# rjagerman/glint

Measured on AMD Instinct MI355X. Metric: device-resident push scatter-add GB/s (and % HBM peak) at 1/2/4/8 GPUs, higher is better.
Workload: dtype f64; 1 GPU; north star: dense contiguous-range push scatter-add, 2^30-key Double vector per GPU (BASELINE.json north_star's 1-GPU target configuration); keys_per_gpu=1073741824, key_dtype=i64, parallelism=range-sharded x1, no exchange

## Files before the change

### glint_amd/csrc/glint_bin.hip

```cpp
#include "glint_device.h"
#include "glint_host.h"

#include <atomic>
#include <cstring>
#include <type_traits>

namespace glint {

#ifndef GLINT_SLAB_BITS
#define GLINT_SLAB_BITS 12
#endif
constexpr int kSlabBits = GLINT_SLAB_BITS;
constexpr int kSlab = 1 << kSlabBits;
constexpr int kMaxDigit = 1024;
#ifndef GLINT_PART_TPB
#define GLINT_PART_TPB 1024
#endif
constexpr int kATPB = GLINT_PART_TPB;
#ifndef GLINT_PART_PER
#define GLINT_PART_PER 4
#endif
constexpr int kAPer = GLINT_PART_PER;
#ifndef GLINT_PART_PER_PLAIN
#define GLINT_PART_PER_PLAIN 8
// ... 264 lines not shown
  const u64 b = ctl->bad;
  if (b == 0ull) {
    if (threadIdx.x == 0) *gate = 0ull;
    return;
  }
  for (u32 x = threadIdx.x; x < nb; x += 256) T[x] = 0;
  if (threadIdx.x == 0) {
    *gate = b;
    ctl->cancel = 1u;
    ctl->brk_enc = 0u;
    bc->tail = 0u;
  }
}

constexpr int kHotSlots = 2048;
constexpr int kHotSample = 16384;
constexpr int kHotRun = 128;
constexpr int kHotRuns = kHotSample / kHotRun;
constexpr int kHotCount = 16384;
constexpr int kHotTPB = 1024;

__device__ __forceinline__ u32 hot_slot(u32 a) { return hot_mix(a) & (kHotSlots - 1); }



template <bool MAT>
__global__ __launch_bounds__(kHotTPB) void bin_hot_pick_kernel(const i64* __restrict__ keys,
                                                               const int32_t* __restrict__ cols, i64 n,
                                                               PartDesc part, const LaunchCtl* lctl, u32 ntiles,
                                                               int from_break, u32 min_count,
                                                               u32* __restrict__ hot_tags) {
  __shared__ u32 ck[kHotCount];
  __shared__ u32 cc[kHotCount];
  __shared__ unsigned long long best[kHotSlots];
  const int tid = threadIdx.x;
  for (int i = tid; i < kHotCount; i += kHotTPB) {
    ck[i] = kEmptySlot;
    cc[i] = 0;
  }
  for (int i = tid; i < kHotSlots; i += kHotTPB) best[i] = 0ull;
  __syncthreads();
  const i64 r0 = tail_start(lctl, ntiles, from_break, n);
  const i64 m = n - r0;
  if (m > 0) {
    const i64 ns = min((i64)kHotSample, m);
    const i64 run_stride = m >= (i64)kHotSample ? m / kHotRuns : kHotRun;
    auto rec_of = [&](i64 sidx) { return r0 + (sidx / kHotRun) * run_stride + (sidx % kHotRun); };
    constexpr int kBatch = 16;
    for (i64 s0 = 0; s0 < ns; s0 += (i64)kBatch * kHotTPB) {
      i64 k[kBatch];
      int32_t c[kBatch];
#pragma unroll
      for (int j = 0; j < kBatch; ++j) {
        const i64 i = rec_of(min(s0 + (i64)j * kHotTPB + tid, ns - 1));
        k[j] = keys[i];
        c[j] = MAT ? cols[i] : 0;
      }
#pragma unroll
      for (int j = 0; j < kBatch; ++j) {
        i64 a64;
        if (s0 + (i64)j * kHotTPB + tid >= ns || !rec_addr<MAT>(part, k[j], c[j], a64)) continue;
        const u32 a = (u32)a64;
        u32 h = hot_mix(a * 0x9E3779B1u) & (kHotCount - 1);
        for (int probe = 0; probe < 64; ++probe) {
          const u32 prev = atomicCAS(&ck[h], kEmptySlot, a);
          if (prev == kEmptySlot || prev == a) {
            atomicAdd(&cc[h], 1u);
            break;
          }
          h = (h + 1) & (kHotCount - 1);
        }
      }
    }
  }
  __syncthreads();
  for (int h = tid; h < kHotCount; h += kHotTPB)
    if (cc[h] >= min_count) atomicMax(&best[hot_slot(ck[h])], ((unsigned long long)cc[h] << 32) | ck[h]);
  __syncthreads();
  for (int i = tid; i < kHotSlots; i += kHotTPB) hot_tags[i] = best[i] ? (u32)best[i] : kEmptySlot;
}

template <typename A> __device__ __forceinline__ A hot_zero() { return A(0); }
template <> __device__ __forceinline__ double hot_zero<double>() { return -0.0; }
template <typename A> __device__ __forceinline__ bool hot_untouched(A x) { return x == A(0); }
template <> __device__ __forceinline__ bool hot_untouched<double>(double x) {
  return __double_as_longlong(x) == (long long)0x8000000000000000ull;
}
__device__ __forceinline__ void hot_flush(double* p, double x) { gadd(p, x); }
__device__ __forceinline__ void hot_flush(float* p, double x) { gadd(p, (float)x); }
__device__ __forceinline__ void hot_flush(long long* p, long long x) { gadd(p, x); }
__device__ __forceinline__ void hot_flush(int* p, int x) { gadd(p, x); }

template <typename A, int P>
__device__ __forceinline__ u32 part_emit(const u32 (&ad)[P], const A (&va)[P], u32 valid, const BinGeom& g,
                                         u32* dcnt, u32* gcnt, u32* st_a, A* st_v, const BufOut& ctb, u32 ctcol,
                                         u32 ctstride, u32* __restrict__ out_a, A* __restrict__ out_v, PhaseClock& ph,
                                         int pb) {
  const int tid = threadIdx.x;
  u32 rank[P];
#pragma unroll
  for (int j = 0; j < P; ++j)
    if (valid & (1u << j)) rank[j] = atomicAdd(&dcnt[bucket_of(ad[j], g)], 1u);
  __syncthreads();
  ph.mark(pb);
  const u32 total = block_scan<kATPB, 1>(
      g.nb, [&](u32 d) { return dcnt[d]; },
      [&](u32 d, u32 excl) {
        gcnt[d] = dcnt[d];
        dcnt[d] = excl;
      });
  ph.mark(pb + 1);
  static_assert(kATPB <= kMaxDigit, "one chunk-table entry per thread");
  bput(ctb, ((u32)tid * ctstride + ctcol) * 4u, (u32)tid < g.nb, dcnt[tid] | (gcnt[tid] << 16));
#pragma unroll
  for (int j = 0; j < P; ++j) {
    if (valid & (1u << j)) {
      const u32 p = dcnt[bucket_of(ad[j], g)] + rank[j];
      st_a[p] = ad[j];
      st_v[p] = va[j];
    }
  }
  __syncthreads();
  ph.mark(pb + 2);
  const RecOut<u32> oa{buf_out(out_a, total * 4u)};
  const RecOut<A> ov{buf_out(out_v, total * (u32)sizeof(A))};
#pragma unroll
  for (int j = 0; j < P; ++j) {
    if ((u32)(j * kATPB) >= total) break;
    const u32 p = tid + j * kATPB;
    const bool on = p < total;
    oa.put(p, on, st_a[p]);
    ov.put(p, on, st_v[p]);
  }
  __syncthreads();
  ph.mark(pb + 3);
  for (u32 d = tid; d < g.nb; d += kATPB) dcnt[d] = 0;
  __syncthreads();
  ph.mark(pb + 4);
  return total;
}

__device__ __forceinline__ void part_next_header(const BinGeom& g, BinCtl* next_bc, u32* __restrict__ next_T,
                                                 LaunchCtl* next_ctl) {
  const int tid = threadIdx.x;
  for (u32 b = tid; b < kMaxDigit; b += kATPB) {
    next_T[b] = 0;
    next_T[kMaxDigit + b] = 0;
  }
  if (tid < (int)(sizeof(BinCtl) / 4)) reinterpret_cast<u32*>(next_bc)[tid] = 0;
  if (next_ctl && tid == 0) {
    next_ctl->brk_enc = 0u;
    next_ctl->nonaffine = 0u;
    next_ctl->cancel = 0u;
    next_ctl->bad = 0ull;
  }
}

__device__ __forceinline__ u32 bucket_items(u32 t, u32 item) { return max(1u, (t + item - 1) / item); }

constexpr int kWideHashBits = 20;
constexpr int kWideRunsPerWg = 8;
constexpr int kWideSampleWgs = 256;

template <bool MAT>
__global__ __launch_bounds__(256) void bin_hot_sample_kernel(const i64* __restrict__ keys, const int32_t* __restrict__ cols,
                                                             i64 n, PartDesc part, const LaunchCtl* lctl, u32 ntiles,
                                                             int from_break, u32* __restrict__ gkey,
                                                             u32* __restrict__ gcnt) {
  constexpr int kLocal = 2048;
  __shared__ u32 lk[kLocal], lc[kLocal];
  const int tid = threadIdx.x;
  for (int i = tid; i < kLocal; i += 256) {
    lk[i] = kEmptySlot;
    lc[i] = 0;
  }
  __syncthreads();
  const i64 r0 = tail_start(lctl, ntiles, from_break, n);
  const i64 m = n - r0;
  const i64 runs = (i64)kWideSampleWgs * kWideRunsPerWg;
  if (m > 0) {
    const i64 stride = m >= runs * kHotRun ? m / runs : kHotRun;
    constexpr int kPer = kWideRunsPerWg * kHotRun / 256;
#pragma unroll
    for (int j = 0; j < kPer; ++j) {
      const int s = j * 256 + tid;
      const i64 run = (i64)blockIdx.x * kWideRunsPerWg + s / kHotRun;
      const i64 i = r0 + run * stride + s % kHotRun;
      if (i >= n) continue;
      i64 a64;
      if (!rec_addr<MAT>(part, keys[i], MAT ? cols[i] : 0, a64)) continue;
      const u32 a = (u32)a64;
      u32 h = hot_mix(a * 0x9E3779B1u) & (kLocal - 1);
      for (int probe = 0; probe < 64; ++probe) {
        const u32 prev = atomicCAS(&lk[h], kEmptySlot, a);
        if (prev == kEmptySlot || prev == a) {
          atomicAdd(&lc[h], 1u);
          break;
        }
        h = (h + 1) & (kLocal - 1);
      }
    }
  }
  __syncthreads();
  constexpr u32 kMask = (1u << kWideHashBits) - 1u;
  for (int i = tid; i < kLocal; i += 256) {
    const u32 a = lk[i];
    if (a == kEmptySlot) continue;
    u32 h = hot_mix(a) & kMask;
    for (int probe = 0; probe < 64; ++probe) {
      const u32 prev = atomicCAS(&gkey[h], kEmptySlot, a);
      if (prev == kEmptySlot || prev == a) {
        atomicAdd(&gcnt[h], lc[i]);
        break;
      }
      h = (h + 1) & kMask;
    }
  }
}

__global__ __launch_bounds__(256) void bin_hot_select_kernel(u32* __restrict__ gkey, u32* __restrict__ gcnt,
                                                             u32 min_count, unsigned long long* __restrict__ best) {
  const u32 i = blockIdx.x * 256u + threadIdx.x;
  const u32 a = gkey[i], c = gcnt[i];
  gkey[i] = kEmptySlot;
  gcnt[i] = 0;
  if (a != kEmptySlot && c >= min_count) atomicMax(&best[wide_slot(a)], ((unsigned long long)c << 32) | a);
}

constexpr int kRedSlots = 64, kRedTPB = 1024, kRedGroups = kRedTPB / kRedSlots;
template <typename V>
__device__ __forceinline__ void hot_reduce_block(u32 blk, const unsigned long long* __restrict__ best, u32 G,
                                                 const typename LdsAcc<V>::T* __restrict__ partial,
                                                 V* __restrict__ data, const LaunchCtl* gated) {
  typedef typename LdsAcc<V>::T A;
  if (gated && gated->cancel) return;
  __shared__ A gs[kRedGroups][kRedSlots];
  __shared__ u32 gany[kRedGroups][kRedSlots];
  const int tid = threadIdx.x, ls = tid % kRedSlots, grp = tid / kRedSlots;
  const u32 sl = blk * (u32)kRedSlots + (u32)ls;
  const u32 per = (G + kRedGroups - 1) / kRedGroups;
  const u32 w0 = grp * per, w1 = min(G, w0 + per);
  A sum = hot_zero<A>();
  u32 any = 0;
  constexpr int kUnroll = 8;
  for (u32 w = w0; w < w1; w += kUnroll) {
    A x[kUnroll];
#pragma unroll
    for (int j = 0; j < kUnroll; ++j) x[j] = partial[(size_t)min(w + (u32)j, w1 - 1u) * kWideSlots + sl];
#pragma unroll
    for (int j = 0; j < kUnroll; ++j) {
      if (w + (u32)j < w1 && !hot_untouched<A>(x[j])) {
        sum = any ? vadd(sum, x[j]) : x[j];
        any = 1;
      }
    }
  }
  gs[grp][ls] = sum;
  gany[grp][ls] = any;
  __syncthreads();
  if (grp != 0) return;
  const unsigned long long b = best[sl];
  if (!b) return;
  A tot = hot_zero<A>();
  bool seen = false;
  for (int q = 0; q < kRedGroups; ++q) {
    if (!gany[q][ls]) continue;
    tot = seen ? vadd(tot, gs[q][ls]) : gs[q][ls];
    seen = true;
  }
  const u32 a = (u32)b;
  if (seen) data[a] = acc_add(data[a], tot);
}

#ifndef GLINT_PART_WAVES
#define GLINT_PART_WAVES 4
#endif
template <typename V, bool MAT, bool HOT, int KIND, bool VALIDATE, int PER = kAPer>
__global__ __launch_bounds__(kATPB) __attribute__((amdgpu_waves_per_eu(HOT ? 4 : GLINT_PART_WAVES))) void bin_part_kernel(
    const i64* __restrict__ keys, const int32_t* __restrict__ cols, const V* __restrict__ vals, i64 n, PartDesc part,
    const LaunchCtl* lctl, u32 ntiles, int from_break, BinGeom g, u32* __restrict__ addr_out,
    typename LdsAcc<V>::T* __restrict__ val_out, ErrState* err, BinCtl* bc, u32* __restrict__ ct, u32 ctstride,
    const unsigned long long* __restrict__ hot_best, typename LdsAcc<V>::T* __restrict__ hot_partial,
    BinCtl* next_bc, u32* __restrict__ next_T, LaunchCtl* vctl, LaunchCtl* next_ctl) {
  typedef typename LdsAcc<V>::T A;
  constexpr int kChunk = kATPB * PER;
  __shared__ u32 dcnt[kMaxDigit], gcnt[kMaxDigit];
  __shared__ u32 st_a[kChunk];
  __shared__ A st_v[kChunk];
  constexpr int kHS = HOT ? kWideSlots : 1;
  __shared__ u32 htag[kHS];
  __shared__ A hacc[kHS];
  const int tid = threadIdx.x;
  const u32 w = blockIdx.x;
  const i64 r0 = tail_start(lctl, ntiles, from_break, n);
  const i64 nchunks = (n - r0 + kChunk - 1) / kChunk;
  constexpr int kAhead = HOT ? 2 : kPartAhead;
  if constexpr (HOT) {
    for (int sl = tid; sl < kWideSlots; sl += kATPB) {
      const unsigned long long b = hot_best[sl];
      htag[sl] = b ? (u32)b : kEmptySlot;
      hacc[sl] = hot_zero<A>();
    }
  }
  for (u32 d = tid; d < g.nb; d += kATPB) dcnt[d] = 0;
  if (w == 0) part_next_header(g, next_bc, next_T, next_ctl);
  __syncthreads();
// ... 1351 lines not shown
```

### glint_amd/csrc/glint_gpu.hip

```cpp
#include "glint_kernels.h"
#include "../../include/glint_gpu.h"
#include "glint_device.h"

#include <mutex>
#include <vector>
#include <utility>
#include <new>
#include <chrono>
#include <cstring>
#include <sched.h>
#include <time.h>
#include <cstdio>
#include <algorithm>
#include <cstdlib>

namespace glint {

template <bool MAT> struct AddrT { typedef int32_t T; };
template <> struct AddrT<true> { typedef i64 T; };

template <bool MAT, int KIND = -1>
__device__ __forceinline__ bool rec_addr_t(const PartDesc& p, i64 key, int32_t col, typename AddrT<MAT>::T& addr) {
  i64 ad;
  const bool ok = rec_addr<MAT, KIND>(p, key, col, ad);
  addr = (typename AddrT<MAT>::T)ad;
  return ok;
}

template <bool MAT, bool FULL, int KIND>
__device__ __forceinline__ bool check_tile(const i64* __restrict__ keys, const int32_t* __restrict__ cols, i64 n,
                                           const PartDesc& part, LaunchCtl* ctl, i64* __restrict__ desc,
                                           u32 ntiles, u32 t, int lane, bool validate, bool read_all) {
  typedef typename AddrT<MAT>::T A;
  const i64 pbase = (i64)t * (kTile / 2);
  K2 k[kPPT];
  C2 c[kPPT];
#pragma unroll
  for (int j = 0; j < kPPT; ++j) {
    const i64 p = pbase + lane + (i64)j * 64;
    const i64 r = 2 * p;
    if (FULL || r + 1 < n) {
      k[j] = __builtin_nontemporal_load(reinterpret_cast<const K2*>(keys) + p);
      if (MAT) c[j] = __builtin_nontemporal_load(reinterpret_cast<const C2*>(cols) + p);
    } else {
      k[j] = K2{r < n ? keys[r] : 0, 0};
      if (MAT) c[j] = C2{r < n ? cols[r] : 0, 0};
    }
  }
  const i64 r_first = 2 * pbase;
  const i64 kb = r_first > 0 ? keys[r_first - 1] : 0;
  const int32_t cb = (MAT && r_first > 0) ? cols[r_first - 1] : 0;
  const u32 brk = __builtin_amdgcn_readfirstlane(ld_relaxed(&ctl->brk_enc));
  const bool after = brk != 0u && ntiles - brk < t;
  if (!read_all && after) return false;
  A before = 0;
  if (r_first > 0) rec_addr_t<MAT, KIND>(part, kb, cb, before);
  bool mono = true, affine = true;
  A a_first = 0;
  A last = before;
#pragma unroll
  for (int j = 0; j < kPPT; ++j) {
    const i64 r = 2 * (pbase + lane + (i64)j * 64);
    const bool h0 = FULL || r < n, h1 = FULL || r + 1 < n;
    A a0, a1;
    const bool o0 = rec_addr_t<MAT, KIND>(part, k[j].x, MAT ? c[j].x : 0, a0);
    const bool o1 = rec_addr_t<MAT, KIND>(part, k[j].y, MAT ? c[j].y : 0, a1);
    if (j == 0) a_first = __shfl(a0, 0);
    if (h1) mono = mono && (a1 > a0);
    A prev = __shfl_up(a1, 1);
    if (lane == 0) prev = last;
    if (h0 && r > 0) mono = mono && (a0 > prev);
    last = __shfl(a1, 63);
    const A off = (A)(r - r_first);
    affine = affine && (!h0 || (o0 && a0 == a_first + off)) && (!h1 || (o1 && a1 == a_first + off + 1));
    if (validate) {
      const bool b0 = h0 && (!o0 || !key_in_part<KIND>(part, k[j].x));
      const bool b1 = h1 && (!o1 || !key_in_part<KIND>(part, k[j].y));
      if (b0 || b1) atomicMax(&ctl->bad, ~(u64)(b0 ? r : r + 1));
    }
  }
  const bool any_bad = __any(!mono);
  const bool all_affine = __all(affine);
  if (lane == 0 && !after) {
    if (any_bad) {
      if (ld_relaxed(&ctl->brk_enc) < ntiles - t) atomicMax(&ctl->brk_enc, ntiles - t);
    } else {
      desc[t] = all_affine ? (i64)a_first : kNotAffine;
      const bool linked = all_affine && (r_first == 0 || (i64)a_first == (i64)before + 1);
      if (!linked && ld_relaxed(&ctl->nonaffine) == 0u) atomicOr(&ctl->nonaffine, 1u);
    }
  }
  return true;
}

template <bool MAT, int KIND>
__global__ __launch_bounds__(kTPB) void push_check_kernel(const i64* __restrict__ keys,
                                                          const int32_t* __restrict__ cols, i64 n,
                                                          PartDesc part, LaunchCtl* ctl, LaunchCtl* next,
                                                          i64* __restrict__ desc, u32 ntiles, u32 t_begin,
                                                          u32 t_end, int validate) {
  const int lane = threadIdx.x & 63;
  if (t_begin == 0 && blockIdx.x == 0 && threadIdx.x == 0) {
    next->brk_enc = 0u;
    next->nonaffine = 0u;
    next->cancel = 0u;
    next->bad = 0ull;
  }
  if (ctl->cancel) return;
  const u32 w0 = blockIdx.x * (kTPB / 64) + (threadIdx.x >> 6);
  const u32 nw = gridDim.x * (kTPB / 64);
  for (u32 t = t_begin + w0; t < t_end; t += nw) {
    const bool full = 2 * ((i64)t * (kTile / 2)) + kTile <= n;
    const bool go = full ? check_tile<MAT, true, KIND>(keys, cols, n, part, ctl, desc, ntiles, t, lane, validate != 0,
                                                       validate == 1)
                         : check_tile<MAT, false, KIND>(keys, cols, n, part, ctl, desc, ntiles, t, lane, validate != 0,
                                                        validate == 1);
    if (!go) return;
  }
}

template <typename V, bool MAT, bool FULL>
__device__ __forceinline__ void apply_affine(const PushArgs<V>& a, i64 pbase, i64 base, int lane) {
  typedef typename Vec2<V>::T V2;
  const i64 n = a.n;
  const i64 r_first = 2 * pbase;
  V2 v[kPPT], d[kPPT];
  if ((base & 1) == 0) {
    V2* dp = reinterpret_cast<V2*>(a.data + base);
#pragma unroll
    for (int j = 0; j < kPPT; ++j) {
      const i64 q = lane + (i64)j * 64;
      if (FULL || 2 * (pbase + q) + 1 < n) {
        v[j] = __builtin_nontemporal_load(reinterpret_cast<const V2*>(a.vals) + pbase + q);
        d[j] = dp[q];
      }
    }
#pragma unroll
    for (int j = 0; j < kPPT; ++j) {
      const i64 q = lane + (i64)j * 64;
      const i64 r = 2 * (pbase + q);
      if (FULL || r + 1 < n) dp[q] = as2<V>(vadd((V)d[j].x, (V)v[j].x), vadd((V)d[j].y, (V)v[j].y));
      else if (r < n) a.data[base + (r - r_first)] = vadd(a.data[base + (r - r_first)], a.vals[r]);
    }
  } else {
#pragma unroll
    for (int j = 0; j < kPPT; ++j) {
      const i64 p = pbase + lane + (i64)j * 64;
      const i64 r = 2 * p;
      const i64 e = base + (r - r_first);
      if (FULL || r + 1 < n) {
        v[j] = __builtin_nontemporal_load(reinterpret_cast<const V2*>(a.vals) + p);
        d[j] = as2<V>(a.data[e], a.data[e + 1]);
      } else {
        v[j] = as2<V>(r < n ? a.vals[r] : V(0), V(0));
        d[j] = as2<V>(r < n ? a.data[e] : V(0), V(0));
      }
    }
#pragma unroll
    for (int j = 0; j < kPPT; ++j) {
      const i64 r = 2 * (pbase + lane + (i64)j * 64);
      const i64 e = base + (r - r_first);
      if (FULL || r < n) a.data[e] = vadd((V)d[j].x, (V)v[j].x);
      if (FULL || r + 1 < n) a.data[e + 1] = vadd((V)d[j].y, (V)v[j].y);
    }
  }
}

template <typename V, bool MAT, bool FULL>
__device__ __forceinline__ void apply_general(const PushArgs<V>& a, i64 pbase, int lane) {
  typedef typename Vec2<V>::T V2;
  typedef typename AddrT<MAT>::T A;
  const i64 n = a.n;
  K2 k[kPPT];
  C2 c[kPPT];
  V2 v[kPPT];
#pragma unroll
  for (int j = 0; j < kPPT; ++j) {
    const i64 p = pbase + lane + (i64)j * 64;
    const i64 r = 2 * p;
    if (FULL || r + 1 < n) {
      k[j] = __builtin_nontemporal_load(reinterpret_cast<const K2*>(a.keys) + p);
      if (MAT) c[j] = __builtin_nontemporal_load(reinterpret_cast<const C2*>(a.cols) + p);
      v[j] = __builtin_nontemporal_load(reinterpret_cast<const V2*>(a.vals) + p);
    } else {
      k[j] = K2{r < n ? a.keys[r] : 0, 0};
      if (MAT) c[j] = C2{r < n ? a.cols[r] : 0, 0};
      v[j] = as2<V>(r < n ? a.vals[r] : V(0), V(0));
    }
  }
#pragma unroll
  for (int j = 0; j < kPPT; ++j) {
    const i64 r = 2 * (pbase + lane + (i64)j * 64);
    A a0, a1;
    const bool h0 = FULL || r < n, h1 = FULL || r + 1 < n;
    const bool o0 = rec_addr_t<MAT>(a.part, k[j].x, MAT ? c[j].x : 0, a0) && h0;
    const bool o1 = rec_addr_t<MAT>(a.part, k[j].y, MAT ? c[j].y : 0, a1) && h1;
    if (h0 && !o0) record_error(a.err, r);
    if (h1 && !o1) record_error(a.err, r + 1);
    if (o0 && o1 && a1 == a0 + 1 && (a0 & 1) == 0) {
      V2* dp = reinterpret_cast<V2*>(a.data + a0);
      const V2 d = *dp;
      *dp = as2<V>(vadd((V)d.x, (V)v[j].x), vadd((V)d.y, (V)v[j].y));
    } else {
      if (o0) a.data[a0] = vadd(a.data[a0], (V)v[j].x);
      if (o1) a.data[a1] = vadd(a.data[a1], (V)v[j].y);
    }
  }
}

constexpr int kSweepU = 2;
template <typename V, bool EVEN>
__device__ __forceinline__ void apply_sweep(const PushArgs<V>& a, i64 delta, i64 p_begin, i64 p_end, bool last) {
  typedef typename Vec2<V>::T V2;
  if (blockIdx.x >= a.sweep_blocks) return;
  const i64 npairs = p_end;
  const i64 stride = (i64)a.sweep_blocks * kTPB;
  const V2* vp = reinterpret_cast<const V2*>(a.vals);
  i64 p = p_begin + (i64)blockIdx.x * kTPB + threadIdx.x;
  if (EVEN) {
    V2* dp = reinterpret_cast<V2*>(a.data + delta);
    for (; p + (kSweepU - 1) * stride < npairs; p += kSweepU * stride) {
      V2 v[kSweepU], d[kSweepU];
#pragma unroll
      for (int j = 0; j < kSweepU; ++j) {
        v[j] = __builtin_nontemporal_load(vp + p + j * stride);
        d[j] = __builtin_nontemporal_load(dp + p + j * stride);
      }
#pragma unroll
      for (int j = 0; j < kSweepU; ++j)
        __builtin_nontemporal_store(as2<V>(vadd((V)d[j].x, (V)v[j].x), vadd((V)d[j].y, (V)v[j].y)), dp + p + j * stride);
    }
    for (; p < npairs; p += stride) {
      const V2 v = __builtin_nontemporal_load(vp + p);
      const V2 d = __builtin_nontemporal_load(dp + p);
      __builtin_nontemporal_store(as2<V>(vadd((V)d.x, (V)v.x), vadd((V)d.y, (V)v.y)), dp + p);
    }
  } else {
    for (; p < npairs; p += stride) {
      const V2 v = __builtin_nontemporal_load(vp + p);
      const i64 e = 2 * p + delta;
      const V d0 = a.data[e], d1 = a.data[e + 1];
      a.data[e] = vadd(d0, (V)v.x);
      a.data[e + 1] = vadd(d1, (V)v.y);
    }
  }
  if ((a.n & 1) && last && blockIdx.x == 0 && threadIdx.x == 0) {
    const i64 e = a.n - 1 + delta;
    a.data[e] = vadd(a.data[e], a.vals[a.n - 1]);
  }
}

template <typename V, bool MAT>
__global__ __launch_bounds__(kTPB) void push_apply_kernel(PushArgs<V> a, const i64* __restrict__ desc, u32 t_begin,
                                                          u32 t_end) {
  if (a.ctl->cancel) return;
  const u32 brk = a.ctl->brk_enc;
  if (t_begin == 0 && blockIdx.x == 0 && threadIdx.x == 0 && a.hint) {
    __hip_atomic_store(a.hint, brk == 0u ? 0ull : (u64)(a.n - (i64)(a.ntiles - brk) * kTile), __ATOMIC_RELAXED,
                       __HIP_MEMORY_SCOPE_SYSTEM);
    __hip_atomic_store(a.hint + 3, brk == 0u ? (u64)a.n : (u64)(a.ntiles - brk) * kTile, __ATOMIC_RELAXED,
                       __HIP_MEMORY_SCOPE_SYSTEM);
  }
  if (brk == 0u && a.ctl->nonaffine == 0u) {
    const i64 delta = desc[0];
    const i64 p0 = (i64)t_begin * (kTile / 2), p1 = min((i64)t_end * (kTile / 2), a.n >> 1);
    const bool last = t_end >= a.ntiles;
    if ((delta & 1) == 0) apply_sweep<V, true>(a, delta, p0, p1, last);
    else apply_sweep<V, false>(a, delta, p0, p1, last);
    return;
  }
  const u32 tiles = min(t_end, brk == 0u ? a.ntiles : a.ntiles - brk);
  const int lane = threadIdx.x & 63;
  const u32 w0 = blockIdx.x * (kTPB / 64) + (threadIdx.x >> 6);
  const u32 nw = gridDim.x * (kTPB / 64);
  i64 dbatch = kNotAffine;
  for (u32 t = t_begin + w0, it = 0; t < tiles; t += nw, ++it) {
    if ((it & 63) == 0) {
      const i64 tt = (i64)t + (i64)lane * nw;
      dbatch = tt < (i64)tiles ? desc[tt] : kNotAffine;
    }
    const i64 pbase = (i64)t * (kTile / 2);
    const i64 base = __shfl(dbatch, (int)(it & 63));
    const bool full = 2 * pbase + kTile <= a.n;
    if (base != kNotAffine) {
      if (full) apply_affine<V, MAT, true>(a, pbase, base, lane);
      else apply_affine<V, MAT, false>(a, pbase, base, lane);
    } else {
      if (full) apply_general<V, MAT, true>(a, pbase, lane);
      else apply_general<V, MAT, false>(a, pbase, lane);
    }
  }
}


constexpr u64 kEmpty = ~0ull;

template <typename V, bool MAT>
__global__ __launch_bounds__(kTPB) void push_scatter_kernel(PushArgs<V> a, int force_all) {
  i64 r0 = 0;
  if (force_all == 2 && blockIdx.x == 0 && threadIdx.x == 0 && a.hint) {
    __hip_atomic_store(a.hint, (u64)a.n, __ATOMIC_RELAXED, __HIP_MEMORY_SCOPE_SYSTEM);
    __hip_atomic_store(a.hint + 3, 0ull, __ATOMIC_RELAXED, __HIP_MEMORY_SCOPE_SYSTEM);
  }
  if (!force_all) {
    const u32 brk = a.ctl->brk_enc;
    if (brk == 0u) return;
    r0 = (i64)(a.ntiles - brk) * kTile;
  }
  if (r0 >= a.n) return;
  const i64 rem = a.n - r0;
  const i64 nchunks = (rem + kScatterChunk - 1) / kScatterChunk;
  if ((i64)blockIdx.x >= nchunks) return;

  typedef typename LdsAcc<V>::T A;
  __shared__ u64 hk[kHashSlots];
  __shared__ A hv[kHashSlots];
  const int tid = threadIdx.x;
  for (int s = tid; s < kHashSlots; s += kTPB) { hk[s] = kEmpty; hv[s] = A(0); }
  __syncthreads();

  for (i64 ch = blockIdx.x; ch < nchunks; ch += gridDim.x) {
    const i64 cbase = r0 + ch * kScatterChunk;
#pragma unroll 2
    for (int q = tid; q < kScatterChunk; q += kTPB) {
      const i64 i = cbase + q;
      if (i >= a.n) break;
      const i64 key = a.keys[i];
      const int32_t col = MAT ? a.cols[i] : 0;
      const V val = a.vals[i];
      i64 addr;
      if (!rec_addr<MAT>(a.part, key, col, addr)) { record_error(a.err, i); continue; }
      const u64 ua = (u64)addr;
      u32 h = (u32)((ua * 0x9E3779B97F4A7C15ull) >> (64 - 12));
      for (;;) {
        const u64 cur = __hip_atomic_load(&hk[h], __ATOMIC_RELAXED, __HIP_MEMORY_SCOPE_WORKGROUP);
        if (cur == ua) break;
        if (cur == kEmpty) {
          const u64 prev = atomicCAS(&hk[h], kEmpty, ua);
          if (prev == kEmpty || prev == ua) break;
        }
        h = (h + 1) & (kHashSlots - 1);
      }
      lds_add(&hv[h], (A)val);
    }
    __syncthreads();
    for (int s = tid; s < kHashSlots; s += kTPB) {
      const u64 key = hk[s];
      if (key != kEmpty) {
        gadd(a.data + key, (V)hv[s]);
        hk[s] = kEmpty;
        hv[s] = A(0);
      }
    }
    __syncthreads();
  }
}

constexpr int kMaxSetShards = 64;
template <typename V>
struct ShardSet {
  int n;
  i64 start[kMaxSetShards];
  i64 end[kMaxSetShards];
  V* data[kMaxSetShards];
};

__device__ __forceinline__ int set_find(const i64* st, const i64* en, int n, i64 key) {
  int lo = 0, hi = n;
  while (lo < hi) {
    const int mid = (lo + hi) >> 1;
    if (st[mid] <= key) lo = mid + 1;
    else hi = mid;
  }
  return lo > 0 && key < en[lo - 1] ? lo - 1 : -1;
}

template <typename V>
__global__ __launch_bounds__(kTPB) void set_validate_kernel(const i64* __restrict__ keys, i64 n, ShardSet<V> set,
                                                            u64* bad) {
  __shared__ i64 st[kMaxSetShards], en[kMaxSetShards];
  if (threadIdx.x < set.n) {
    st[threadIdx.x] = set.start[threadIdx.x];
    en[threadIdx.x] = set.end[threadIdx.x];
  }
  __syncthreads();
  u64 b = 0;
  if (((uintptr_t)keys & 15) == 0) {
    typedef __attribute__((ext_vector_type(2))) long long KP;
    const i64 np = n >> 1, stride = (i64)gridDim.x * kTPB;
    i64 p = (i64)blockIdx.x * kTPB + threadIdx.x;
    for (; p + 3 * stride < np; p += 4 * stride) {
      KP k[4];
#pragma unroll
      for (int u = 0; u < 4; ++u) k[u] = __builtin_nontemporal_load(reinterpret_cast<const KP*>(keys) + p + u * stride);
#pragma unroll
      for (int u = 0; u < 4; ++u) {
        const i64 i = 2 * (p + u * stride);
        if (set_find(st, en, set.n, k[u].y) < 0) b = max(b, ~(u64)(i + 1));
        if (set_find(st, en, set.n, k[u].x) < 0) b = max(b, ~(u64)i);
      }
    }
    for (; p < np; p += stride) {
      const KP k = __builtin_nontemporal_load(reinterpret_cast<const KP*>(keys) + p);
      if (set_find(st, en, set.n, k.y) < 0) b = max(b, ~(u64)(2 * p + 1));
      if (set_find(st, en, set.n, k.x) < 0) b = max(b, ~(u64)(2 * p));
    }
    if ((n & 1) && blockIdx.x == 0 && threadIdx.x == 0 && set_find(st, en, set.n, keys[n - 1]) < 0)
      b = max(b, ~(u64)(n - 1));
  } else {
    const i64 stride = (i64)gridDim.x * kTPB;
    for (i64 i = (i64)blockIdx.x * kTPB + threadIdx.x; i < n; i += stride)
      if (set_find(st, en, set.n, keys[i]) < 0) b = max(b, ~(u64)i);
  }
  for (int d = 32; d > 0; d >>= 1) b = max(b, (u64)__shfl_xor((unsigned long long)b, d));
  if ((threadIdx.x & 63) == 0 && b) atomicMax((unsigned long long*)bad, (unsigned long long)b);
}

__global__ void set_gate_kernel(const u64* bad, u64* gate) {
  if (threadIdx.x == 0) *gate = *bad;
}

template <typename V>
__global__ __launch_bounds__(kTPB) void set_scatter_kernel(const i64* __restrict__ keys, const V* __restrict__ vals,
                                                           i64 n, ShardSet<V> set, const u64* bad) {
  if (*bad != 0ull) return;
  const i64 nchunks = (n + kScatterChunk - 1) / kScatterChunk;
  typedef typename LdsAcc<V>::T A;
  __shared__ u64 hk[kHashSlots];
  __shared__ A hv[kHashSlots];
  __shared__ i64 st[kMaxSetShards], en[kMaxSetShards];
  __shared__ V* dp[kMaxSetShards];
  const int tid = threadIdx.x;
  if (tid < set.n) {
    st[tid] = set.start[tid];
    en[tid] = set.end[tid];
    dp[tid] = set.data[tid];
  }
  for (int q = tid; q < kHashSlots; q += kTPB) { hk[q] = kEmpty; hv[q] = A(0); }
  __syncthreads();
  for (i64 ch = blockIdx.x; ch < nchunks; ch += gridDim.x) {
    const i64 cbase = ch * kScatterChunk;
#pragma unroll 2
    for (int q = tid; q < kScatterChunk; q += kTPB) {
// ... 145 lines not shown
      int lo = 0, hi = nm - 1;
      while (lo < hi) {
        const int mid = (lo + hi + 1) >> 1;
        if ((i64)s_off[mid] <= r) lo = mid;
        else hi = mid - 1;
      }
      s_dst[lo][r - (i64)s_off[lo]] = v[j];
    }
  } else {
#pragma unroll
    for (int j = 0; j < kRingPullPer; ++j) {
      const i64 r = (i64)j * kRingPullTPB + threadIdx.x;
      if (j < per && r < n) out[r] = v[j];
    }
  }
  msg_signal(sig, err);
}

template <typename V>
__global__ __launch_bounds__(kTPB) void mat_pull_kernel(const i64* rows, const int32_t* cols, i64 n, const V* data,
                                                        PartDesc part, V* out, ErrState* err, MsgSig sig) {
  for (i64 i = (i64)blockIdx.x * kTPB + threadIdx.x; i < n; i += (i64)gridDim.x * kTPB) {
    i64 ad;
    const bool o = rec_addr<true>(part, rows[i], cols[i], ad);
    if (!o) record_error(err, i);
    out[i] = o ? data[ad] : V(0);
  }
  msg_signal(sig, err);
}

template <typename V, bool VEC16>
__global__ __launch_bounds__(kTPB) void mat_pull_rows_kernel(const i64* rows, i64 n, const V* data, PartDesc part,
                                                             V* out, ErrState* err, MsgSig sig) {
  const int lane = threadIdx.x & 63;
  const i64 w0 = (i64)blockIdx.x * (kTPB / 64) + (threadIdx.x >> 6);
  const i64 nw = (i64)gridDim.x * (kTPB / 64);
  const i64 cols = part.cols;
  for (i64 i = w0; i < n; i += nw) {
    const int32_t l = g2l(part, rows[i]);
    const bool ok = l >= 0 && l < part.size;
    if (!ok && lane == 0) record_error(err, i);
    if (VEC16) {
      typedef __attribute__((ext_vector_type(4))) unsigned int U4;
      const i64 chunks = cols * (i64)sizeof(V) / 16;
      const U4* src = reinterpret_cast<const U4*>(data + (ok ? (i64)l : 0) * part.pitch);
      U4* dst = reinterpret_cast<U4*>(out + i * cols);
#pragma unroll 4
      for (i64 c = lane; c < chunks; c += 64) dst[c] = ok ? src[c] : U4{0, 0, 0, 0};
    } else {
      const V* src = data + (ok ? (i64)l : 0) * part.pitch;
      V* dst = out + i * cols;
      for (i64 c = lane; c < cols; c += 64) dst[c] = ok ? src[c] : V(0);
    }
  }
  msg_signal(sig, err);
}

}

using namespace glint;

#include "glint_host.h"

namespace {

constexpr int kSweepBlocksPerCu = 1;

constexpr u32 kSweepWindowTiles = ((u32)1 << 26) / kTile;

int binned_mode() {
  static EnvKnob k("GLINT_BINNED");
  return (int)k.get([](const char* e) -> long long {
    if (!e || !*e) return -1;
    return atoi(e) != 0 ? 1 : 0;
  });
}
constexpr i64 kBinMin = (i64)1 << 20;
i64 bin_density() {
  static EnvKnob k("GLINT_BIN_DENSITY");
  return k.get([](const char* e) -> long long { return e ? std::max(0ll, atoll(e)) : 512ll; });
}
constexpr i64 kSmallPushMax = 4096;

template <typename V, bool MAT>
int launch_push(glint_shard* s, const i64* keys, const int32_t* cols, const void* vals, i64 n, int flags,
                hipStream_t st) {
  if (n <= 0) return GLINT_OK;
  if (!keys || !vals || (MAT && !cols)) return GLINT_EINVAL;
  PushArgs<V> a;
  a.keys = keys;
  a.cols = cols;
  a.vals = (const V*)vals;
  a.n = n;
  a.data = (V*)s->data;
  a.part = s->part;
  a.err = err_of(s);
  a.elems = s->elems;
  a.hint = s->d_hint;
  a.sig = s->sig;
  a.sweep_blocks = 0;
  const i64 ntiles = (n + kTile - 1) / kTile;
  if (ntiles >= (i64)0xFFFFFFF0ll) return GLINT_EINVAL;
  a.ntiles = (u32)ntiles;
  const bool vec_ok = aligned(keys, 16) && aligned(vals, 2 * sizeof(V)) && (!MAT || aligned(cols, 8));
  const bool fp = s->dtype == GLINT_F32 || s->dtype == GLINT_F64;
  const bool det = (flags & GLINT_PUSH_DETERMINISTIC) && fp;
  const bool unordered = (flags & GLINT_PUSH_UNORDERED) != 0;
  const bool seq = det || (fp && (flags & kPushHostSequential) && !unordered);
  const bool gated = s->gate != nullptr;
  if (gated && (det || !vec_ok)) return GLINT_EINVAL;
  if (a.sig.done || (seq && n <= kOrderedMax && s->elems < ((i64)1 << 32))) return push_ordered<V, MAT>(s, a, st);
  const size_t ctl_need = 256 + (size_t)ntiles * sizeof(i64);
  const void* ctl_old = s->d_ctl;
  int rc = grow(&s->d_ctl, &s->ctl_bytes, ctl_need);
  if (rc) return rc;
  if (s->d_ctl != ctl_old) {
    HIPCHK(hipMemsetAsync(s->d_ctl, 0, 2 * sizeof(LaunchCtl), st));
    s->ctl_par = 0;
  }
  LaunchCtl* const slots = (LaunchCtl*)s->d_ctl;
  a.ctl = slots + s->ctl_par;
  i64* desc = (i64*)((char*)s->d_ctl + 256);

  const int bmode = binned_mode();
  const i64 last_tail = (i64)s->hint_tail;
  const i64 slabs = (s->elems + 4095) / 4096;
  const bool binned = !det && vec_ok && push_binnable(s, n) && bmode != 0 &&
                      (unordered || (n >= kBinMin && (bmode == 1 || (last_tail >= kBinMin &&
                                                                     last_tail >= bin_density() * slabs))));
  if (binned && unordered && !gated) return push_binned<V, MAT>(s, a, false, st);
  const bool validate = gated && (flags & GLINT_PUSH_VALIDATE) != 0;
  static EnvKnob whole_knob("GLINT_BIN_WHOLE");
  const bool whole = binned && (!gated || validate) && s->hint_tail > 0 && s->hint_head == 0 &&
                     whole_knob.get([](const char* e) -> long long { return e ? atoi(e) != 0 : 1; }) != 0;
  if (whole) {
    LaunchCtl* const next = slots + (s->ctl_par ^ 1);
    const BinHook hook = [&](void* bc, u32* T, u32 nb) -> int {
      return launch_validate_gate_binned(a.ctl, s->gate, bc, T, nb, st);
    };
    rc = push_binned<V, MAT>(s, a, false, st, validate ? &hook : nullptr, next);
    if (rc == GLINT_OK) s->ctl_par ^= 1;
    return rc;
  }
  const bool small = !det && !gated && n <= kSmallPushMax;
  const bool whole_scatter = !binned && !det && !gated && vec_ok && !small && s->hint_tail > 0 &&
                             s->hint_head == 0 && (s->whole_probe++ & 7u) != 7u &&
                             whole_knob.get([](const char* e) -> long long { return e ? atoi(e) != 0 : 1; }) != 0;
  if (!vec_ok || small || whole_scatter) {
    if (det) return push_det_tail<V, MAT>(s, a, false, st);
    const unsigned g2 = grid_for(n, kScatterChunk, (i64)s->cus * 2);
    HIPCHK(launch_k(s, GLINT_K_PUSH_SCATTER, push_scatter_kernel<V, MAT>, g2, kTPB, st, a, whole_scatter ? 2 : 1));
    return GLINT_OK;
  }
  const u64 win = std::min<u64>(kSweepWindowTiles, a.ntiles);
  const bool fuse = validate && binned && !det;
  {
    LaunchCtl* const next = slots + (s->ctl_par ^ 1);
    if (gated && !validate) {
      push_gate_kernel<<<1, 64, 0, st>>>(s->gate, a.ctl);
      HIPCHK(hipGetLastError());
    }
    const unsigned gc =
        grid_for(a.ntiles, kTPB / 64, (i64)s->cus * blocks_per_cu<push_check_kernel<MAT, 0>>(2));
    HIPCHK(a.part.kind == 0 ? launch_k(s, GLINT_K_PUSH_CHECK, push_check_kernel<MAT, 0>, gc, kTPB, st, keys, cols, n,
                                       a.part, a.ctl, next, desc, a.ntiles, 0u, a.ntiles, validate ? (fuse ? 2 : 1) : 0)
                            : launch_k(s, GLINT_K_PUSH_CHECK, push_check_kernel<MAT, 1>, gc, kTPB, st, keys, cols, n,
                                       a.part, a.ctl, next, desc, a.ntiles, 0u, a.ntiles, validate ? (fuse ? 2 : 1) : 0));
    if (validate && !fuse) {
      push_validate_gate_kernel<<<1, 64, 0, st>>>(a.ctl, s->gate);
      HIPCHK(hipGetLastError());
    }
    s->ctl_par ^= 1;
  }
  auto apply_head = [&]() -> int {
    const i64 bpc = blocks_per_cu<push_apply_kernel<V, MAT>>(2);
    for (u64 t0 = 0; t0 < a.ntiles; t0 += win) {
      const u32 t1 = (u32)std::min<u64>(a.ntiles, t0 + win);
      const unsigned ga = grid_for(t1 - t0, kTPB / 64, (i64)s->cus * bpc);
      a.sweep_blocks = std::min<u32>(ga, (u32)((i64)s->cus * kSweepBlocksPerCu));
      HIPCHK(launch_k(s, GLINT_K_PUSH_APPLY, push_apply_kernel<V, MAT>, ga, kTPB, st, a, (const i64*)desc, (u32)t0, t1));
    }
    return GLINT_OK;
  };
  if (fuse) {
    const BinHook hook = [&](void* bc, u32* T, u32 nb) -> int {
      const int rc2 = launch_validate_gate_binned(a.ctl, s->gate, bc, T, nb, st);
      return rc2 ? rc2 : apply_head();
    };
    return push_binned<V, MAT>(s, a, true, st, &hook);
  }
  rc = apply_head();
  if (rc) return rc;
  if (det) return push_det_tail<V, MAT>(s, a, true, st);
  if (binned) return push_binned<V, MAT>(s, a, true, st);
  const unsigned g2 = grid_for(n, kScatterChunk, (i64)s->cus * 2);
  HIPCHK(launch_k(s, GLINT_K_PUSH_SCATTER, push_scatter_kernel<V, MAT>, g2, kTPB, st, a, 0));
  return GLINT_OK;
}

template <typename V>
int launch_vec_pull(glint_shard* s, const i64* keys, void* out, i64 n, hipStream_t st) {
  if (n <= 0) return GLINT_OK;
  if (!keys || !out) return GLINT_EINVAL;
  const MsgSig sig = s->sig;
  if (sig.done && n <= kRingPullMax) {
    HIPCHK(launch_k(s, GLINT_K_VEC_PULL, ring_pull_kernel<V, false>, 1u, kRingPullTPB, st, keys, (const int32_t*)nullptr,
                    n, (const V*)s->data, s->part, (V*)out, err_of(s), sig, s->pull_tab, s->pull_nm));
    return GLINT_OK;
  }
  const bool pairs = aligned(keys, 16) && aligned(out, 2 * sizeof(V));
  if (pairs) {
    const i64 npairs = (n + 1) / 2;
    const i64 win = sig.done ? npairs : std::min<i64>(npairs, (i64)kSweepWindowTiles * (kTile / 2));
    for (i64 p0 = 0; p0 < npairs; p0 += win) {
      const i64 p1 = std::min<i64>(npairs, p0 + win);
      const unsigned g = sig.done ? 1u : grid_for(p1 - p0, kTPB, (i64)s->cus * kPullBlocksPerCu);
      HIPCHK(launch_k(s, GLINT_K_VEC_PULL, vec_pull_kernel<V, true>, g, kTPB, st, keys, n, (const V*)s->data, s->part,
                      (V*)out, err_of(s), sig, p0, p1));
    }
  } else {
    const unsigned g = sig.done ? 1u : grid_for(n, kTPB, (i64)s->cus * 8);
    HIPCHK(launch_k(s, GLINT_K_VEC_PULL, vec_pull_kernel<V, false>, g, kTPB, st, keys, n, (const V*)s->data, s->part,
                    (V*)out, err_of(s), sig, (i64)0, (i64)0));
  }
  return GLINT_OK;
}

template <typename V>
int launch_mat_pull(glint_shard* s, const i64* rows, const int32_t* cols, void* out, i64 n, hipStream_t st) {
  if (n <= 0) return GLINT_OK;
  if (!rows || !cols || !out) return GLINT_EINVAL;
  const MsgSig sig = s->sig;
  if (sig.done && n <= kRingPullMax) {
    HIPCHK(launch_k(s, GLINT_K_MAT_PULL, ring_pull_kernel<V, true>, 1u, kRingPullTPB, st, rows, cols, n,
                    (const V*)s->data, s->part, (V*)out, err_of(s), sig, s->pull_tab, s->pull_nm));
    return GLINT_OK;
  }
  const unsigned g = sig.done ? 1u : grid_for(n, kTPB, (i64)s->cus * 8);
  HIPCHK(launch_k(s, GLINT_K_MAT_PULL, mat_pull_kernel<V>, g, kTPB, st, rows, cols, n, (const V*)s->data, s->part,
                  (V*)out, err_of(s), sig));
  return GLINT_OK;
}

template <typename V>
int launch_mat_pull_rows(glint_shard* s, const i64* rows, void* out, i64 n, hipStream_t st) {
  if (n <= 0) return GLINT_OK;
  if (!rows || !out) return GLINT_EINVAL;
  const MsgSig sig = s->sig;
  const bool v16 = ((i64)s->part.cols * (i64)sizeof(V)) % 16 == 0 && aligned(out, 16);
  const unsigned g = sig.done ? 1u : grid_for(n, kTPB / 64, (i64)s->cus * 8);
  HIPCHK(launch_k(s, GLINT_K_MAT_PULL_ROWS, v16 ? mat_pull_rows_kernel<V, true> : mat_pull_rows_kernel<V, false>, g,
                  kTPB, st, rows, n, (const V*)s->data, s->part, (V*)out, err_of(s), sig));
  return GLINT_OK;
}

#define GLINT_DISPATCH(dt, FN, ...)                            \
  switch (dt) {                                                \
    case GLINT_F64: return FN<double>(__VA_ARGS__);            \
    case GLINT_F32: return FN<float>(__VA_ARGS__);             \
    case GLINT_I64: return FN<long long>(__VA_ARGS__);         \
    case GLINT_I32: return FN<int>(__VA_ARGS__);               \
    default: return GLINT_EINVAL;                              \
  }

template <typename V>
int push_vec_t(glint_shard* s, const i64* k, const int32_t*, const void* v, i64 n, int f, hipStream_t st) {
  return launch_push<V, false>(s, k, nullptr, v, n, f, st);
}
template <typename V>
int push_mat_t(glint_shard* s, const i64* k, const int32_t* c, const void* v, i64 n, int f, hipStream_t st) {
  return launch_push<V, true>(s, k, c, v, n, f, st);
}

template <typename V>
int launch_set_push(glint_shard* const* sh, int m, const i64* keys, const void* vals, i64 n, u64* gate,
                    hipStream_t st) {
  glint_shard* s0 = sh[0];
  ShardSet<V> set{};
  set.n = m;
  for (int j = 0; j < m; ++j) {
    set.start[j] = sh[j]->part.start;
    set.end[j] = sh[j]->part.start + sh[j]->part.size;
    set.data[j] = (V*)sh[j]->data;
  }
  u64* word = nullptr;
  for (auto& sw : s0->set_words)
    if (sw.first == st) word = sw.second;
  if (!word) {
    if (hipMalloc((void**)&word, sizeof(u64)) != hipSuccess) {
      (void)hipGetLastError();
      return GLINT_ENOMEM;
    }
    s0->set_words.emplace_back(st, word);
  }
  HIPCHK(hipMemsetAsync(word, 0, sizeof(u64), st));
  const unsigned gv = grid_for(n, (i64)kTPB * 16, (i64)s0->cus * 4);
  HIPCHK(launch_k(s0, GLINT_K_PUSH_CHECK, set_validate_kernel<V>, gv, kTPB, st, keys, n, set, word));
  set_gate_kernel<<<1, 64, 0, st>>>(word, gate);
  HIPCHK(hipGetLastError());
  const unsigned g2 = grid_for(n, kScatterChunk, (i64)s0->cus * 2);
  HIPCHK(launch_k(s0, GLINT_K_PUSH_SCATTER, set_scatter_kernel<V>, g2, kTPB, st, keys, (const V*)vals, n, set,
                  (const u64*)word));
  return GLINT_OK;
}

int create_common(glint_shard* s, int device, int dtype, int32_t cols, void* view_data = nullptr) {
  if (dtype < GLINT_I32 || dtype > GLINT_F64 || cols < 0) return GLINT_EINVAL;
  static EnvKnob hprof_knob("GLINT_HOST_PROF");
  s->hprof = hprof_knob.pos_or(0) != 0;
  if (s->part.size < 0) return GLINT_EINVAL;
  int ndev = 0;
  if (hipGetDeviceCount(&ndev) != hipSuccess || device < 0 || device >= ndev) {
    (void)hipGetLastError();
    return GLINT_EDEVICE;
  }
  DeviceGuard g(device);
  if (!g.ok) return GLINT_EDEVICE;
  s->device = device;
  s->dtype = dtype;
  s->vsize = dtype_size(dtype);
  s->part.cols = cols;
  const i64 per16 = 16 / (i64)s->vsize;
  s->part.pitch = cols > 0 ? ((i64)cols + per16 - 1) / per16 * per16 : 1;
  s->elems = cols > 0 ? (i64)s->part.size * s->part.pitch : (i64)s->part.size;
  hipDeviceProp_t prop;
  if (hipGetDeviceProperties(&prop, device) == hipSuccess && prop.multiProcessorCount > 0)
    s->cus = prop.multiProcessorCount;
  HIPCHK(hipStreamCreateWithFlags(&s->stream, hipStreamNonBlocking));
  const size_t bytes = (size_t)s->elems * s->vsize + 16;
  if (view_data) {
    s->data = view_data;
  } else if (hipMalloc(&s->data, bytes) != hipSuccess) {
    (void)hipGetLastError();
    return GLINT_ENOMEM;
// ... 1603 lines not shown
```

### glint_amd/csrc/glint_kernels.h

```cpp
#pragma once
#include <hip/hip_runtime.h>
#include <stdint.h>

namespace glint {

typedef long long i64;
typedef unsigned long long u64;
typedef unsigned int u32;

constexpr int kTPB = 256;
constexpr int kPPT = 8;
constexpr int kTile = 64 * kPPT * 2;
constexpr i64 kNotAffine = (i64)0x8000000000000000ll;
constexpr int kHashSlots = 4096;
constexpr int kScatterChunk = 2048;
constexpr i64 kOrderedMax = (i64)1 << 17;
constexpr int kPushHostSequential = 1 << 16;

struct LaunchCtl {
  u32 brk_enc;
  u32 nonaffine;
  u32 cancel;
  u32 pad_;
  u64 bad;
};

struct ErrState {
  u64 min_bad_enc;
  u64 count;
};

struct MsgSig {
  u64* done;
  u64 ticket;
  ErrState* herr;
};

struct PullDst {
  unsigned int off, n;
  unsigned long long dst;
};
constexpr int kPullDirectMax = 256;

struct PartDesc {
  int32_t kind;
  int32_t size;
  int64_t start;
  int32_t cidx;
  int32_t cparts;
  int32_t cols;
  int32_t pad_;
  int64_t pitch;
};

template <int KIND = -1>
__device__ __forceinline__ int32_t g2l(const PartDesc& p, i64 key) {
  if (KIND == 0 || (KIND < 0 && p.kind == 0)) return (int32_t)(key - p.start);
  return (int32_t)((key - (i64)p.cidx) / (i64)p.cparts);
}

template <typename V>
struct PushArgs {
  const i64* keys;
  const int32_t* cols;
  const V* vals;
  i64 n;
  V* data;
  i64 elems;
  PartDesc part;
  LaunchCtl* ctl;
  u32 ntiles;
  ErrState* err;
  u32 sweep_blocks;
  u64* hint;
  MsgSig sig;
};

}
```

Baseline: 6322 GB/s.

## Replace windowed apply launches with single ticket-scheduled persistent apply kernel

```diff
diff --git a/glint_amd/csrc/glint_bin.hip b/glint_amd/csrc/glint_bin.hip
--- a/glint_amd/csrc/glint_bin.hip
+++ b/glint_amd/csrc/glint_bin.hip
@@ -440,6 +440,7 @@
     next_ctl->brk_enc = 0u;
     next_ctl->nonaffine = 0u;
     next_ctl->cancel = 0u;
+    next_ctl->ticket = 0u;
     next_ctl->bad = 0ull;
   }
 }
diff --git a/glint_amd/csrc/glint_gpu.hip b/glint_amd/csrc/glint_gpu.hip
--- a/glint_amd/csrc/glint_gpu.hip
+++ b/glint_amd/csrc/glint_gpu.hip
@@ -104,6 +104,7 @@
     next->brk_enc = 0u;
     next->nonaffine = 0u;
     next->cancel = 0u;
+    next->ticket = 0u;
     next->bad = 0ull;
   }
   if (ctl->cancel) return;
@@ -209,86 +210,124 @@
 }
 
 constexpr int kSweepU = 2;
-template <typename V, bool EVEN>
-__device__ __forceinline__ void apply_sweep(const PushArgs<V>& a, i64 delta, i64 p_begin, i64 p_end, bool last) {
+template <typename V, bool EVEN, class Took>
+__device__ __forceinline__ void apply_sweep(const PushArgs<V>& a, i64 delta, i64 p0, i64 p1, int lane, Took took) {
   typedef typename Vec2<V>::T V2;
-  if (blockIdx.x >= a.sweep_blocks) return;
-  const i64 npairs = p_end;
-  const i64 stride = (i64)a.sweep_blocks * kTPB;
   const V2* vp = reinterpret_cast<const V2*>(a.vals);
-  i64 p = p_begin + (i64)blockIdx.x * kTPB + threadIdx.x;
   if (EVEN) {
     V2* dp = reinterpret_cast<V2*>(a.data + delta);
-    for (; p + (kSweepU - 1) * stride < npairs; p += kSweepU * stride) {
+    auto step = [&](i64 p) {
       V2 v[kSweepU], d[kSweepU];
 #pragma unroll
       for (int j = 0; j < kSweepU; ++j) {
-        v[j] = __builtin_nontemporal_load(vp + p + j * stride);
-        d[j] = __builtin_nontemporal_load(dp + p + j * stride);
+        v[j] = __builtin_nontemporal_load(vp + p + j * 64);
+        d[j] = __builtin_nontemporal_load(dp + p + j * 64);
       }
 #pragma unroll
       for (int j = 0; j < kSweepU; ++j)
-        __builtin_nontemporal_store(as2<V>(vadd((V)d[j].x, (V)v[j].x), vadd((V)d[j].y, (V)v[j].y)), dp + p + j * stride);
-    }
-    for (; p < npairs; p += stride) {
-      const V2 v = __builtin_nontemporal_load(vp + p);
-      const V2 d = __builtin_nontemporal_load(dp + p);
-      __builtin_nontemporal_store(as2<V>(vadd((V)d.x, (V)v.x), vadd((V)d.y, (V)v.y)), dp + p);
+        __builtin_nontemporal_store(as2<V>(vadd((V)d[j].x, (V)v[j].x), vadd((V)d[j].y, (V)v[j].y)), dp + p + j * 64);
+    };
+    auto rest = [&](i64 p) {
+      for (; p + (kSweepU - 1) * 64 < p1; p += kSweepU * 64) step(p);
+      for (; p < p1; p += 64) {
+        const V2 v = __builtin_nontemporal_load(vp + p);
+        const V2 d = __builtin_nontemporal_load(dp + p);
+        __builtin_nontemporal_store(as2<V>(vadd((V)d.x, (V)v.x), vadd((V)d.y, (V)v.y)), dp + p);
+      }
+    };
+    if (p0 + kSweepU * 64 <= p1) {
+      step(p0 + lane);
+      took();
+      rest(p0 + kSweepU * 64 + lane);
+    } else {
+      rest(p0 + lane);
+      took();
     }
   } else {
-    for (; p < npairs; p += stride) {
+    auto step = [&](i64 p) {
       const V2 v = __builtin_nontemporal_load(vp + p);
       const i64 e = 2 * p + delta;
       const V d0 = a.data[e], d1 = a.data[e + 1];
       a.data[e] = vadd(d0, (V)v.x);
       a.data[e + 1] = vadd(d1, (V)v.y);
-    }
-  }
-  if ((a.n & 1) && last && blockIdx.x == 0 && threadIdx.x == 0) {
-    const i64 e = a.n - 1 + delta;
-    a.data[e] = vadd(a.data[e], a.vals[a.n - 1]);
+    };
+    i64 p = p0 + lane;
+    if (p0 + 64 <= p1) {
+      step(p);
+      p += 64;
+      took();
+      for (; p < p1; p += 64) step(p);
+    } else {
+      if (p < p1) step(p);
+      took();
+    }
   }
 }
 
 template <typename V, bool MAT>
-__global__ __launch_bounds__(kTPB) void push_apply_kernel(PushArgs<V> a, const i64* __restrict__ desc, u32 t_begin,
-                                                          u32 t_end) {
+__global__ __launch_bounds__(kTPB) void push_apply_kernel(PushArgs<V> a, const i64* __restrict__ desc) {
   if (a.ctl->cancel) return;
   const u32 brk = a.ctl->brk_enc;
-  if (t_begin == 0 && blockIdx.x == 0 && threadIdx.x == 0 && a.hint) {
+  if (blockIdx.x == 0 && threadIdx.x == 0 && a.hint) {
     __hip_atomic_store(a.hint, brk == 0u ? 0ull : (u64)(a.n - (i64)(a.ntiles - brk) * kTile), __ATOMIC_RELAXED,
                        __HIP_MEMORY_SCOPE_SYSTEM);
     __hip_atomic_store(a.hint + 3, brk == 0u ? (u64)a.n : (u64)(a.ntiles - brk) * kTile, __ATOMIC_RELAXED,
                        __HIP_MEMORY_SCOPE_SYSTEM);
   }
-  if (brk == 0u && a.ctl->nonaffine == 0u) {
-    const i64 delta = desc[0];
-    const i64 p0 = (i64)t_begin * (kTile / 2), p1 = min((i64)t_end * (kTile / 2), a.n >> 1);
-    const bool last = t_end >= a.ntiles;
-    if ((delta & 1) == 0) apply_sweep<V, true>(a, delta, p0, p1, last);
-    else apply_sweep<V, false>(a, delta, p0, p1, last);
-    return;
-  }
-  const u32 tiles = min(t_end, brk == 0u ? a.ntiles : a.ntiles - brk);
+  const bool sweep = brk == 0u && a.ctl->nonaffine == 0u;
+  const u32 nb = sweep ? a.sweep_blocks : gridDim.x;
+  if (blockIdx.x >= nb) return;
+  const u32 tiles = brk == 0u ? a.ntiles : a.ntiles - brk;
+  const bool large = a.ntiles > (u32)kApplyPieceTiles * 8u * nb;
+  const u32 pt = large ? (u32)kApplyPieceTiles
+                       : a.ntiles > (u32)kApplyPieceTiles * nb ? (u32)kApplyPieceTiles / 4
+                                                               : ((a.ntiles + nb - 1) / nb + 3u) & ~3u;
+  const u32 pt_end = large ? (u32)kApplyPieceTiles / 4 : pt;
+  const u32 whole = large ? (tiles / pt > nb ? tiles / pt - nb : 0u) : (tiles + pt - 1) / pt;
+  const u32 npieces = large ? whole + (tiles - whole * pt + pt_end - 1) / pt_end : whole;
+  const bool ticketed = npieces > nb;
   const int lane = threadIdx.x & 63;
-  const u32 w0 = blockIdx.x * (kTPB / 64) + (threadIdx.x >> 6);
-  const u32 nw = gridDim.x * (kTPB / 64);
-  i64 dbatch = kNotAffine;
-  for (u32 t = t_begin + w0, it = 0; t < tiles; t += nw, ++it) {
-    if ((it & 63) == 0) {
-      const i64 tt = (i64)t + (i64)lane * nw;
-      dbatch = tt < (i64)tiles ? desc[tt] : kNotAffine;
-    }
-    const i64 pbase = (i64)t * (kTile / 2);
-    const i64 base = __shfl(dbatch, (int)(it & 63));
-    const bool full = 2 * pbase + kTile <= a.n;
-    if (base != kNotAffine) {
-      if (full) apply_affine<V, MAT, true>(a, pbase, base, lane);
-      else apply_affine<V, MAT, false>(a, pbase, base, lane);
+  const u32 wave = __builtin_amdgcn_readfirstlane((int)(threadIdx.x >> 6));
+  const i64 delta = sweep ? desc[0] : 0;
+  if (sweep && (a.n & 1) && blockIdx.x == 0 && threadIdx.x == 0) {
+    const i64 e = a.n - 1 + delta;
+    a.data[e] = vadd(a.data[e], a.vals[a.n - 1]);
+  }
+  __shared__ u32 s_next[2];
+  u32 nv = 0;
+  u32 t = blockIdx.x;
+  for (u32 it = 0; t < npieces; ++it) {
+    if (ticketed && threadIdx.x == 0) nv = atomicInc(&a.ctl->ticket, 0xFFFFFFFFu);
+    auto took = [&] {
+      if (ticketed && threadIdx.x == 0) s_next[it & 1] = nv;
+    };
+    const u32 wt = (t < whole ? pt : pt_end) / (kTPB / 64);
+    const i64 t0 = (t < whole ? (i64)t * pt : (i64)whole * pt + (i64)(t - whole) * pt_end) + wave * wt;
+    const i64 t1 = min(t0 + (i64)wt, (i64)tiles);
+    if (sweep) {
+      const i64 p0 = t0 * (kTile / 2), p1 = min(t1 * (kTile / 2), a.n >> 1);
+      if ((delta & 1) == 0) apply_sweep<V, true>(a, delta, p0, p1, lane, took);
+      else apply_sweep<V, false>(a, delta, p0, p1, lane, took);
     } else {
-      if (full) apply_general<V, MAT, true>(a, pbase, lane);
-      else apply_general<V, MAT, false>(a, pbase, lane);
-    }
+      const i64 dbatch = t0 + lane < t1 ? desc[t0 + lane] : kNotAffine;
+      for (i64 tt = t0; tt < t1; ++tt) {
+        const i64 pbase = tt * (kTile / 2);
+        const i64 base = __shfl(dbatch, (int)(tt - t0));
+        const bool full = 2 * pbase + kTile <= a.n;
+        if (base != kNotAffine) {
+          if (full) apply_affine<V, MAT, true>(a, pbase, base, lane);
+          else apply_affine<V, MAT, false>(a, pbase, base, lane);
+        } else {
+          if (full) apply_general<V, MAT, true>(a, pbase, lane);
+          else apply_general<V, MAT, false>(a, pbase, lane);
+        }
+        if (tt == t0) took();
+      }
+      if (t0 >= t1) took();
+    }
+    if (!ticketed) break;
+    __syncthreads();
+    t = nb + s_next[it & 1];
   }
 }
 
@@ -740,7 +779,6 @@
     HIPCHK(launch_k(s, GLINT_K_PUSH_SCATTER, push_scatter_kernel<V, MAT>, g2, kTPB, st, a, whole_scatter ? 2 : 1));
     return GLINT_OK;
   }
-  const u64 win = std::min<u64>(kSweepWindowTiles, a.ntiles);
   const bool fuse = validate && binned && !det;
   {
     LaunchCtl* const next = slots + (s->ctl_par ^ 1);
@@ -762,12 +800,9 @@
   }
   auto apply_head = [&]() -> int {
     const i64 bpc = blocks_per_cu<push_apply_kernel<V, MAT>>(2);
-    for (u64 t0 = 0; t0 < a.ntiles; t0 += win) {
-      const u32 t1 = (u32)std::min<u64>(a.ntiles, t0 + win);
-      const unsigned ga = grid_for(t1 - t0, kTPB / 64, (i64)s->cus * bpc);
-      a.sweep_blocks = std::min<u32>(ga, (u32)((i64)s->cus * kSweepBlocksPerCu));
-      HIPCHK(launch_k(s, GLINT_K_PUSH_APPLY, push_apply_kernel<V, MAT>, ga, kTPB, st, a, (const i64*)desc, (u32)t0, t1));
-    }
+    const unsigned ga = grid_for(a.ntiles, kTPB / 64, (i64)s->cus * bpc);
+    a.sweep_blocks = std::min<u32>(ga, (u32)((i64)s->cus * kSweepBlocksPerCu));
+    HIPCHK(launch_k(s, GLINT_K_PUSH_APPLY, push_apply_kernel<V, MAT>, ga, kTPB, st, a, (const i64*)desc));
     return GLINT_OK;
   };
   if (fuse) {
diff --git a/glint_amd/csrc/glint_kernels.h b/glint_amd/csrc/glint_kernels.h
--- a/glint_amd/csrc/glint_kernels.h
+++ b/glint_amd/csrc/glint_kernels.h
@@ -11,6 +11,7 @@
 constexpr int kTPB = 256;
 constexpr int kPPT = 8;
 constexpr int kTile = 64 * kPPT * 2;
+constexpr int kApplyPieceTiles = 16;
 constexpr i64 kNotAffine = (i64)0x8000000000000000ll;
 constexpr int kHashSlots = 4096;
 constexpr int kScatterChunk = 2048;
@@ -21,7 +22,7 @@
   u32 brk_enc;
   u32 nonaffine;
   u32 cancel;
-  u32 pad_;
+  u32 ticket;
   u64 bad;
 };
 
```

After: 6314 GB/s. About the same (-0.1%).
